# openclimatefix/predict_pv_yield

Measured on AMD Instinct MI355X. Metric: PV-site samples/sec (train step), conv3d 12->6 frames, higher is better.
Workload: dtype bf16; 1 GPU; conv3d train step (fwd + NMAE + bwd + Adam): sat [B,11,18,64,64] N(0,1), 4x Conv3d(3x3x3, 32ch) + fc 128/128/64, 128.6 M params; per_gpu_batch=32, global_batch=32, t_frames=18, parallelism=single

## Files before the change

predict_pv_yield_amd/csrc/conv3d_wgrad_bf16_v2.hip:

```cpp
#include "pv_common.h"

namespace pv {

constexpr int W2TR = 8, W2TRI = 10, W2TW = 32, W2XW = 34;
constexpr int W2_SLAB_ELEMS = 28 * 32 * 32;
constexpr uint32_t W2_INVALID = 0x40000000u;

typedef __attribute__((address_space(3))) s16x4 w2_lds_s16x4;
typedef __attribute__((address_space(3))) unsigned char* w2_lds_ptr;
typedef int w2_i32x4 __attribute__((ext_vector_type(4)));

__device__ __forceinline__ void w2_lds_dma16(uint32_t lds_addr, uint32_t voff, w2_i32x4 rsrc, uint32_t soff) {
  asm volatile("s_mov_b32 m0, %0\n\ts_nop 0\n\tbuffer_load_dwordx4 %1, %2, %3 offen lds" ::"s"(lds_addr), "v"(voff), "s"(rsrc),
               "s"(soff)
               : "memory");
}
__device__ __forceinline__ w2_i32x4 w2_rsrc(const void* base, int bytes) {
  const uintptr_t a = (uintptr_t)base;
  return (w2_i32x4){(int)(uint32_t)a, (int)((a >> 32) & 0xffffu), bytes, 0x00020000};
}

#ifdef PV_DIAG_STAMPS
__device__ unsigned long long wgrad2_diag[PV_DIAG_WAVES * PV_DIAG_SLOTS];
#endif

template <int NACC, int Q>
__device__ __forceinline__ void w2_interleave() {
  if constexpr (Q < NACC) {
    constexpr int R = 2 + 2 * NACC;
    __builtin_amdgcn_sched_group_barrier(0x008, 1, 0);
    __builtin_amdgcn_sched_group_barrier(0x100, R / NACC + (Q < R % NACC ? 1 : 0), 0);
    w2_interleave<NACC, Q + 1>();
  }
}

template <int CPAD, bool F16 = false, bool PACK12 = false>
__global__ __launch_bounds__(512, 2) void conv3d_wgrad_bf16_v2_kernel(
    const uint16_t* __restrict__ x, const uint16_t* __restrict__ dy, float* __restrict__ slabs, int t_in, int h_in, int w_in,
    int t_out, int h_out, int w_out, int pad_t, int pad_h, int pad_w, int n_colblk, int t_chunk, int rpb) {
  constexpr int NCH = CPAD / 8;
  constexpr int VPR = 16 / NCH;
  constexpr int VOXB = CPAD * 2;
  constexpr int ROWB = W2XW * VOXB;
  constexpr int SLOTB = W2TRI * ROWB;
  constexpr int XVPP = 1024 / VOXB;
  constexpr int XPIECES = (W2XW + XVPP - 1) / XVPP;
  constexpr int XTAIL_LANES = (W2XW - (XPIECES - 1) * XVPP) * NCH;
  constexpr int DROWB = W2TW * 64;
  constexpr int DSLOTB = W2TR * DROWB;
  constexpr int NXS = 5;
  __shared__ __attribute__((aligned(1024))) unsigned char lds[NXS * SLOTB + 256 + 2 * DSLOTB];
  unsigned char* lds_const = lds + NXS * SLOTB;
  unsigned char* lds_dy = lds_const + 256;

  const int tid = threadIdx.x;
  const int lane = tid & 63;
  const int wave8 = __builtin_amdgcn_readfirstlane(tid >> 6);
  const bool loader = wave8 >= 4;
  const int wave = wave8 & 3;
  const int grp = lane >> 4;
  const int qi = (lane & 15) >> 2;
  const int pi = lane & 3;
  const int hh = grp >> 1;
  const int cb = 16 * (grp & 1);

  const int h0 = blockIdx.x * rpb;
  const int b = blockIdx.z;
  const int tc0 = blockIdx.y * t_chunk;
  const int tc1 = min(tc0 + t_chunk, t_out);
  const int wg_id = (blockIdx.z * gridDim.y + blockIdx.y) * gridDim.x + blockIdx.x;
  float* slab = slabs + (size_t)wg_id * W2_SLAB_ELEMS;

  static_assert(!PACK12 || CPAD == 16, "PACK12 packs the 16-channel image");
  constexpr bool PAIRED = CPAD == 16;
  constexpr int NACC = PACK12 ? 3 : (PAIRED ? 4 : 7);
  f32x16 acc[NACC];
#pragma unroll
  for (int i = 0; i < NACC; ++i)
#pragma unroll
    for (int j = 0; j < 16; ++j) acc[i][j] = 0.f;

  const int nt = tc1 - tc0, tn = nt + 2;
  const int n_items = nt > 0 ? nt * n_colblk : 0;
  const int u_end = tn * n_colblk;
  const uint32_t lds_base = __builtin_amdgcn_readfirstlane((uint32_t)(uintptr_t)(w2_lds_ptr)lds);

  if (n_items > 0 && loader) {
    const uint32_t x_plane_b = (uint32_t)h_in * w_in * CPAD * 2u, x_row_b = (uint32_t)w_in * CPAD * 2u;
    const uint32_t d_plane_b = (uint32_t)h_out * w_out * 64u, d_row_b = (uint32_t)w_out * 64u;
    const size_t x_sample = (size_t)t_in * h_in * w_in * CPAD, d_sample = (size_t)t_out * h_out * w_out * 32;
    const void* const x_base = x + (size_t)b * x_sample;
    const void* const d_base = dy + (size_t)b * d_sample;
    const int x_bytes = (int)(x_sample * 2), d_bytes = (int)(d_sample * 2);
    uint32_t xrow_src[3];
    bool xrow_in[3];
#pragma unroll
    for (int i = 0; i < 3; ++i) {
      const int hi = h0 - pad_h + wave + 4 * i;
      xrow_in[i] = (unsigned)hi < (unsigned)h_in && wave + 4 * i < rpb + 2;
      xrow_src[i] = xrow_in[i] ? (uint32_t)hi * x_row_b : 0u;
    }
    uint32_t drow_src[2];
    bool drow_in[2];
#pragma unroll
    for (int i = 0; i < 2; ++i) {
      const int ho = h0 + wave + 4 * i;
      drow_in[i] = ho < h_out && wave + 4 * i < rpb;
      drow_src[i] = drow_in[i] ? (uint32_t)ho * d_row_b : 0u;
    }
    const bool has_third_row = wave + 8 < W2TRI;
    auto x_slice = [&](int u) {
      const int cb = u / tn, s = tc0 + (u - cb * tn), w0 = cb * W2TW;
      const int ti = s - pad_t;
      const bool t_ok = (unsigned)ti < (unsigned)t_in;
      const uint32_t slot = lds_base + (uint32_t)((u % NXS) * SLOTB);
#pragma unroll
      for (int pc = 0; pc < XPIECES; ++pc) {
        const int v = pc * XVPP + lane / NCH;
        const int src = (lane % NCH) ^ ((v / VPR) % NCH);
        const int wi = w0 - pad_w + v;
        const uint32_t lane_off = ((unsigned)wi < (unsigned)w_in && v < W2XW) ? (uint32_t)(wi * CPAD + src * 8) * 2u : W2_INVALID;
#pragma unroll
        for (int i = 0; i < 3; ++i) {
          if (i == 2 && !has_third_row) continue;
          const bool ok = t_ok && xrow_in[i];
          if (pc + 1 < XPIECES || lane < XTAIL_LANES)
            w2_lds_dma16(slot + (uint32_t)((wave + 4 * i) * ROWB + pc * 1024), lane_off, w2_rsrc(x_base, ok ? x_bytes : 0),
                         ok ? (uint32_t)ti * x_plane_b + xrow_src[i] : 0u);
        }
      }
    };
    auto d_slice = [&](int v_seq) {
      const int cb = v_seq / nt, t = tc0 + (v_seq - cb * nt), w0 = cb * W2TW;
      const uint32_t slot = lds_base + (uint32_t)(NXS * SLOTB + 256 + (v_seq & 1) * DSLOTB);
#pragma unroll
      for (int pc = 0; pc < 2; ++pc) {
        const int v = pc * 16 + (lane >> 2);
        const int src = (lane & 3) ^ ((v >> 2) & 3);
        const uint32_t lane_off = (w0 + v) < w_out ? (uint32_t)((w0 + v) * 32 + src * 8) * 2u : W2_INVALID;
#pragma unroll
        for (int i = 0; i < 2; ++i) {
          const bool ok = drow_in[i];
          w2_lds_dma16(slot + (uint32_t)((wave + 4 * i) * DROWB + pc * 1024), lane_off, w2_rsrc(d_base, ok ? d_bytes : 0),
                       ok ? (uint32_t)t * d_plane_b + drow_src[i] : 0u);
        }
      }
    };

    int next_u = 0;
    for (; next_u < 4 && next_u < u_end; ++next_u) x_slice(next_u);
    d_slice(0);
    for (int j = 0; j < n_items; ++j) {
      const int cb = j / nt, u0 = cb * tn + (j - cb * nt);
      __builtin_amdgcn_s_waitcnt(0x0f70);
      __syncthreads();
      if (next_u < u0 + 3) {
        for (; next_u < u0 + 3; ++next_u) x_slice(next_u);
        __builtin_amdgcn_s_waitcnt(0x0f70);
        __syncthreads();
      }
      for (; next_u <= u0 + 4 && next_u < u_end; ++next_u) x_slice(next_u);
      if (j + 1 < n_items) d_slice(j + 1);
    }
  } else if (n_items > 0) {
    if (tid < 64) reinterpret_cast<uint32_t*>(lds_const)[tid] = tid < 32 ? (F16 ? 0x3c003c00u : 0x3f803f80u) : 0u;

    int aoff[2];
#pragma unroll
    for (int s = 0; s < 2; ++s) {
      const int v = 8 * hh + 4 * s + qi;
      const int chunk = (cb + 4 * pi) >> 3;
      aoff[s] = v * 64 + ((chunk ^ ((v >> 2) & 3)) << 4) + (pi & 1) * 8;
    }
    int boff[NACC][2];
    int bkt[NACC];
    int my_tap[NACC];
#pragma unroll
    for (int i = 0; i < NACC; ++i) {
      int tap, c4 = 0;
      if constexpr (PACK12) {
        const int piece = 8 * (wave + 4 * i) + 4 * (grp & 1) + pi;
        tap = piece / 3;
        c4 = piece - 3 * tap;
        if (piece > 81) tap = 28;
      } else {
        tap = PAIRED ? 2 * (wave + 4 * i) + (grp & 1) : wave + 4 * i;
      }
      my_tap[i] = tap;
      if (tap > 26) tap = 26;
      const int kt = tap / 9, kh = (tap / 3) % 3, kw = tap % 3;
      bkt[i] = kt;
      const int cbx = PAIRED ? 0 : cb;
#pragma unroll
      for (int s = 0; s < 2; ++s) {
        const int v = kw + 8 * hh + 4 * s + qi;
        const int chunk = PACK12 ? (c4 >> 1) : ((cbx + 4 * pi) >> 3);
        const int sub = PACK12 ? (c4 & 1) : (pi & 1);
        boff[i][s] = kh * ROWB + v * VOXB + ((chunk ^ ((v / VPR) % NCH)) << 4) + sub * 8;
      }
    }
    typedef __attribute__((ext_vector_type(8))) short s16x8;
    const int last_tap = (PAIRED || PACK12) ? my_tap[NACC - 1] : (wave == 3 ? 27 : 0);
    const unsigned char* const_frag = last_tap < 27 ? nullptr : lds_const + (last_tap == 27 ? 0 : 128) + (lane & 15) * 8;

#ifdef PV_DIAG_STAMPS
    unsigned long long dg[PV_DIAG_SLOTS] = {0, 0, 0, 0, 0, 0, 0, 0}, s0, s1, s2;
#endif
    for (int j = 0; j < n_items; ++j) {
      const int cbj = j / nt, u0 = cbj * tn + (j - cbj * nt);
      PV_STAMP(s0);
      __syncthreads();
      if (cbj > 0 && j == cbj * nt) __syncthreads();
      PV_STAMP(s1);
      int slot_of_kt[3];
#pragma unroll
      for (int kt = 0; kt < 3; ++kt) slot_of_kt[kt] = ((u0 + kt) % NXS) * SLOTB;
      const unsigned char* dy_slot = lds_dy + (j & 1) * DSLOTB;
      int bslot[NACC];
#pragma unroll
      for (int i = 0; i < NACC; ++i) bslot[i] = bkt[i] == 0 ? slot_of_kt[0] : (bkt[i] == 1 ? slot_of_kt[1] : slot_of_kt[2]);
      auto read_step = [&](int st, s16x4 (&ra)[2], s16x4 (&rb)[NACC][2]) {
        const int rho = st >> 1, cg = st & 1;
        const unsigned char* ap = dy_slot + rho * DROWB + cg * 16 * 64;
        ra[0] = __builtin_amdgcn_ds_read_tr16_b64_v4i16((w2_lds_s16x4*)(ap + aoff[0]));
        ra[1] = __builtin_amdgcn_ds_read_tr16_b64_v4i16((w2_lds_s16x4*)(ap + aoff[1]));
        const int xo = rho * ROWB + cg * 16 * VOXB;
#pragma unroll
        for (int i = 0; i < NACC; ++i) {
          const unsigned char* bp = lds + bslot[i] + xo;
          const unsigned char* p0 = bp + boff[i][0];
          const unsigned char* p1 = bp + boff[i][1];
          if (i == NACC - 1) {
            p0 = const_frag ? const_frag : p0;
            p1 = const_frag ? const_frag : p1;
          }
          rb[i][0] = __builtin_amdgcn_ds_read_tr16_b64_v4i16((w2_lds_s16x4*)p0);
          rb[i][1] = __builtin_amdgcn_ds_read_tr16_b64_v4i16((w2_lds_s16x4*)p1);
        }
      };
      auto mfma_step = [&](const s16x4 (&ra)[2], const s16x4 (&rb)[NACC][2]) {
        const s16x8 a8 = {ra[0][0], ra[0][1], ra[0][2], ra[0][3], ra[1][0], ra[1][1], ra[1][2], ra[1][3]};
        typedef _Float16 w2_f16x8 __attribute__((ext_vector_type(8)));
#pragma unroll
        for (int i = 0; i < NACC; ++i) {
          s16x8 t8 = {rb[i][0][0], rb[i][0][1], rb[i][0][2], rb[i][0][3], rb[i][1][0], rb[i][1][1], rb[i][1][2], rb[i][1][3]};
          if constexpr (F16)
            acc[i] = __builtin_amdgcn_mfma_f32_32x32x16_f16(__builtin_bit_cast(w2_f16x8, a8), __builtin_bit_cast(w2_f16x8, t8), acc[i], 0, 0, 0);
          else
            acc[i] = __builtin_amdgcn_mfma_f32_32x32x16_bf16(__builtin_bit_cast(bf16x8, a8), __builtin_bit_cast(bf16x8, t8), acc[i], 0, 0, 0);
        }
      };
      s16x4 ra0[2], ra1[2], rb0[NACC][2], rb1[NACC][2];
      const bool skip_last_row = rpb < W2TR;
      read_step(0, ra0, rb0);
#pragma unroll
      for (int st = 0; st < W2TR * 2; st += 2) {
        if (st == W2TR * 2 - 2 && skip_last_row) break;
        __builtin_amdgcn_sched_barrier(0);
        read_step(st + 1, ra1, rb1);
        mfma_step(ra0, rb0);
        w2_interleave<NACC, 0>();
        __builtin_amdgcn_sched_barrier(0);
        if (st + 2 < W2TR * 2) {
          read_step(st + 2, ra0, rb0);
          mfma_step(ra1, rb1);
          w2_interleave<NACC, 0>();
        } else {
          mfma_step(ra1, rb1);
        }
        __builtin_amdgcn_sched_barrier(0);
      }
#ifdef PV_DIAG_STAMPS
      PV_STAMP(s2);
      dg[0] += s1 - s0;
      dg[1] += s2 - s1;
      dg[2] += 1;
#endif
    }
#ifdef PV_DIAG_STAMPS
    if (lane == 0 && wg_id * 4 + wave < PV_DIAG_WAVES)
      for (int i = 0; i < PV_DIAG_SLOTS; ++i) wgrad2_diag[(size_t)(wg_id * 4 + wave) * PV_DIAG_SLOTS + i] = dg[i];
#endif
  }
  if (loader) return;

  const int half = lane >> 5;
#pragma unroll
  for (int i = 0; i < NACC; ++i) {
    int tapslot = PAIRED ? 2 * (wave + 4 * i) + ((lane & 31) >> 4) : wave + 4 * i;
    int ci = PAIRED ? (lane & 15) : (lane & 31);
    if constexpr (PACK12) {
      const int piece = 8 * (wave + 4 * i) + ((lane & 31) >> 2);
      tapslot = piece / 3;
      ci = 4 * (piece - 3 * tapslot) + (lane & 3);
      if (piece > 81) tapslot = 28;
    }
    if (tapslot <= 27) {
      float* dst = slab + (size_t)tapslot * 1024 + ci;
#pragma unroll
      for (int j = 0; j < 16; ++j) {
        const int co = (j & 3) + 8 * (j >> 2) + 4 * half;
        dst[co * 32] = acc[i][j];
      }
    }
  }
}

void wgrad_v2_grid(const pv_conv3d_dims* d, int* n_rowblk, int* n_colblk, int* n_tchunk, int* t_chunk, int* rows_per_blk) {
  const int to = d->t_in + 2 * d->pad_t - 2, ho = d->h_in + 2 * d->pad_h - 2, wo = d->w_in + 2 * d->pad_w - 2;
  *n_rowblk = (ho + W2TR - 1) / W2TR;
  if ((long long)d->batch * *n_rowblk < 256 && (long long)d->batch * (*n_rowblk + 1) <= 256 &&
      (ho + *n_rowblk) / (*n_rowblk + 1) < (ho + *n_rowblk - 1) / *n_rowblk)
    *n_rowblk += 1;
  *rows_per_blk = (ho + *n_rowblk - 1) / *n_rowblk;
  *n_colblk = (wo + W2TW - 1) / W2TW;
  const long long tiles = (long long)d->batch * *n_rowblk;
  int max_chunks = (to + 1) / 2;
  if (max_chunks < 1) max_chunks = 1;
  int ntc = 1;
  long long best = -1;
  for (int c = 1; c <= max_chunks && tiles * c <= 16 * 256; ++c) {
    const int tch = (to + c - 1) / c, nch = (to + tch - 1) / tch;
    const long long rounds = (tiles * nch + 255) / 256;
    const long long cost = rounds * (tch + 2);
    if (best < 0 || cost < best) best = cost, ntc = nch;
  }
  *t_chunk = (to + ntc - 1) / ntc;
  *n_tchunk = (to + *t_chunk - 1) / *t_chunk;
}

size_t wgrad_v2_workspace_bytes(const pv_conv3d_dims* d) {
  int nrb, ncb, ntc, tch, rpb;
  wgrad_v2_grid(d, &nrb, &ncb, &ntc, &tch, &rpb);
  return (size_t)d->batch * nrb * ntc * W2_SLAB_ELEMS * sizeof(float);
}

int launch_conv3d_wgrad_bf16_v2(const uint16_t* x, const uint16_t* dy, float* slabs, const pv_conv3d_dims* d, int to, int ho,
                                int wo, hipStream_t st, int* n_slabs, bool f16) {
  if (((uintptr_t)x % 16) != 0 || ((uintptr_t)dy % 16) != 0) return 1;
  int nrb, ncb, ntc, tch, rpb;
  wgrad_v2_grid(d, &nrb, &ncb, &ntc, &tch, &rpb);
  *n_slabs = d->batch * nrb * ntc;
  dim3 grid((unsigned)nrb, (unsigned)ntc, (unsigned)d->batch);
#define PV_W2(CP, HALF)                                                                                                       \
  hipLaunchKernelGGL((conv3d_wgrad_bf16_v2_kernel<CP, HALF>), grid, dim3(512), 0, st, x, dy, slabs, d->t_in, d->h_in, d->w_in, to, \
                     ho, wo, d->pad_t, d->pad_h, d->pad_w, ncb, tch, rpb)
#define PV_W2P(HALF)                                                                                                        \
  hipLaunchKernelGGL((conv3d_wgrad_bf16_v2_kernel<16, HALF, true>), grid, dim3(512), 0, st, x, dy, slabs, d->t_in, d->h_in, d->w_in, \
                     to, ho, wo, d->pad_t, d->pad_h, d->pad_w, ncb, tch, rpb)
  if (pv_bf16_cpad(d->c_in) == 16) {
    const bool pack12 = d->c_in <= 12 && !getenv("PV_WGRAD_NO_PACK12");
    if (pack12) { if (f16) PV_W2P(true); else PV_W2P(false); }
    else { if (f16) PV_W2(16, true); else PV_W2(16, false); }
  } else { if (f16) PV_W2(32, true); else PV_W2(32, false); }
#undef PV_W2P
#undef PV_W2
  return 0;
}


constexpr int WR_GROUPS = 16;
__global__ __launch_bounds__(64 * WR_GROUPS) void conv3d_wgrad_reduce_kernel(const float* __restrict__ slabs, int n_slabs,
                                                                              float* __restrict__ dw, float* __restrict__ dbias,
                                                                              int c_out, int c_in) {
  __shared__ float part[WR_GROUPS][64];
  const int lane = threadIdx.x & 63, grp = threadIdx.x >> 6;
  const int i = blockIdx.x * 64 + lane;
  float s0 = 0.f, s1 = 0.f, s2 = 0.f, s3 = 0.f;
  for (int k = grp; k < n_slabs; k += 16 * WR_GROUPS) {
    float v[16];
#pragma unroll
    for (int j = 0; j < 16; ++j) v[j] = (k + WR_GROUPS * j < n_slabs) ? slabs[(size_t)(k + WR_GROUPS * j) * W2_SLAB_ELEMS + i] : 0.f;
#pragma unroll
    for (int j = 0; j < 16; j += 4) s0 += v[j], s1 += v[j + 1], s2 += v[j + 2], s3 += v[j + 3];
  }
  part[grp][lane] = (s0 + s1) + (s2 + s3);
  __syncthreads();
  if (grp == 0) {
    float t[WR_GROUPS];
#pragma unroll
    for (int q = 0; q < WR_GROUPS; ++q) t[q] = part[q][lane];
#pragma unroll
    for (int w = WR_GROUPS / 2; w >= 1; w >>= 1)
#pragma unroll
      for (int q = 0; q < w; ++q) t[q] = t[2 * q] + t[2 * q + 1];
    const float s = t[0];
    const int tap = i >> 10, co = (i >> 5) & 31, ci = i & 31;
    if (tap < 27) {
      if (dw && co < c_out && ci < c_in) dw[((size_t)co * c_in + ci) * 27 + tap] = s;
    } else if (dbias && ci == 0 && co < c_out) {
      dbias[co] = s;
    }
  }
}

__global__ __launch_bounds__(256) void wgrad_gate_copy_kernel(const u32x4* __restrict__ dy, const u32x4* __restrict__ y,
                                                              u32x4* __restrict__ dst, size_t n8) {
  const size_t stride = (size_t)gridDim.x * blockDim.x;
  for (size_t i = (size_t)blockIdx.x * blockDim.x + threadIdx.x; i < n8; i += stride) {
    const u32x4 g = dy[i], a = y[i];
    u32x4 o;
#pragma unroll
    for (int j = 0; j < 4; ++j) o[j] = g[j] & (relu_pair01(a[j]) * 0xffffu);
    dst[i] = o;
  }
}

}

using namespace pv;

extern "C" {

int pv_conv3d_bwd_weight_bf16_workspace_bytes(const pv_conv3d_dims* d, size_t* bytes) {
  PV_REQUIRE(d && bytes, PV_EINVAL, "pv_conv3d_bwd_weight_bf16_workspace_bytes: null pointer");
  PV_REQUIRE(d->batch > 0 && d->t_in > 0 && d->h_in > 0 && d->w_in > 0, PV_EINVAL,
             "pv_conv3d_bwd_weight_bf16_workspace_bytes: bad dims");
  const long long to = d->t_in + 2 * d->pad_t - 2, ho = d->h_in + 2 * d->pad_h - 2, wo = d->w_in + 2 * d->pad_w - 2;
  const size_t dy_bytes = (to > 0 && ho > 0 && wo > 0) ? (size_t)d->batch * to * ho * wo * pv_bf16_cpad(d->c_out) * 2 : 0;
  *bytes = ((wgrad_v2_workspace_bytes(d) + 255) & ~(size_t)255) + dy_bytes;
  return PV_OK;
}

int pv_conv3d_bwd_weight_bf16(const uint16_t* x, const uint16_t* dy, const uint16_t* y_relu_mask, float* dw,
                              float* dbias, const pv_conv3d_dims* d, void* workspace, size_t workspace_bytes,
                              void* stream) {
  PV_REQUIRE(d && x && dy && workspace, PV_EINVAL, "pv_conv3d_bwd_weight_bf16: null pointer");
  PV_REQUIRE(d->batch > 0 && d->c_in > 0 && d->c_in <= 32 && d->c_out > 0 && d->c_out <= 32, PV_ESIZE,
             "pv_conv3d_bwd_weight_bf16: channels (%d -> %d) must be in 1..32", d->c_in, d->c_out);
  PV_REQUIRE(d->pad_t >= 0 && d->pad_t <= 2 && d->pad_h >= 0 && d->pad_h <= 2 && d->pad_w >= 0 && d->pad_w <= 2,
             PV_EINVAL, "pv_conv3d_bwd_weight_bf16: padding must be 0..2");
  const int to = d->t_in + 2 * d->pad_t - 2, ho = d->h_in + 2 * d->pad_h - 2, wo = d->w_in + 2 * d->pad_w - 2;
  PV_REQUIRE(to > 0 && ho > 0 && wo > 0, PV_ESIZE, "pv_conv3d_bwd_weight_bf16: input smaller than the kernel");
  PV_REQUIRE(d->batch <= 65535, PV_ESIZE, "pv_conv3d_bwd_weight_bf16: batch too large for grid.z");
  PV_REQUIRE((size_t)d->t_in * d->h_in * d->w_in * 64 <= 0x40000000ull, PV_ESIZE,
             "pv_conv3d_bwd_weight_bf16: one sample exceeds 1 GiB (buffer-addressing limit of this kernel)");
  const size_t slab_bytes = (wgrad_v2_workspace_bytes(d) + 255) & ~(size_t)255;
  PV_REQUIRE(workspace_bytes >= wgrad_v2_workspace_bytes(d), PV_ESIZE, "pv_conv3d_bwd_weight_bf16: workspace too small");
  PV_REQUIRE(((uintptr_t)x % 16) == 0 && ((uintptr_t)dy % 16) == 0 && ((uintptr_t)workspace % 16) == 0, PV_EINVAL,
             "pv_conv3d_bwd_weight_bf16: x, dy and the workspace must be 16-byte aligned");
  hipStream_t st = as_stream(stream);
  if (y_relu_mask) {
    const size_t n = (size_t)d->batch * to * ho * wo * pv_bf16_cpad(d->c_out);
    PV_REQUIRE(workspace_bytes >= slab_bytes + n * 2, PV_ESIZE,
               "pv_conv3d_bwd_weight_bf16: a gate needs room for the gated copy of dY behind the slabs (workspace_bytes query)");
    PV_REQUIRE(((uintptr_t)y_relu_mask % 16) == 0, PV_EINVAL, "pv_conv3d_bwd_weight_bf16: the gate must be 16-byte aligned");
    uint16_t* gated = reinterpret_cast<uint16_t*>(static_cast<char*>(workspace) + slab_bytes);
    hipLaunchKernelGGL(wgrad_gate_copy_kernel, dim3(stream_grid(n / 8, 256)), dim3(256), 0, st,
                       reinterpret_cast<const u32x4*>(dy), reinterpret_cast<const u32x4*>(y_relu_mask),
                       reinterpret_cast<u32x4*>(gated), n / 8);
    dy = gated;
  }
  int n2 = 0;
  PV_REQUIRE(launch_conv3d_wgrad_bf16_v2(x, dy, (float*)workspace, d, to, ho, wo, st, &n2, false) == 0, PV_EINVAL,
             "pv_conv3d_bwd_weight_bf16: x and dy must be 16-byte aligned");
  hipLaunchKernelGGL(conv3d_wgrad_reduce_kernel, dim3(W2_SLAB_ELEMS / 64), dim3(64 * WR_GROUPS), 0, st, (const float*)workspace, n2,
                     dw, dbias, d->c_out, d->c_in);
  return check_launch("pv_conv3d_bwd_weight_bf16");
}

int pv_conv3d_bwd_weight_f16(const uint16_t* x, const uint16_t* dy, float* dw, float* dbias, const pv_conv3d_dims* d,
                             void* workspace, size_t workspace_bytes, void* stream) {
  PV_REQUIRE(d && x && dy && workspace, PV_EINVAL, "pv_conv3d_bwd_weight_f16: null pointer");
  PV_REQUIRE(d->batch > 0 && d->c_in > 0 && d->c_in <= 32 && d->c_out > 0 && d->c_out <= 32, PV_ESIZE,
             "pv_conv3d_bwd_weight_f16: channels (%d -> %d) must be in 1..32", d->c_in, d->c_out);
  PV_REQUIRE(d->pad_t >= 0 && d->pad_t <= 2 && d->pad_h >= 0 && d->pad_h <= 2 && d->pad_w >= 0 && d->pad_w <= 2,
             PV_EINVAL, "pv_conv3d_bwd_weight_f16: padding must be 0..2");
  const int to = d->t_in + 2 * d->pad_t - 2, ho = d->h_in + 2 * d->pad_h - 2, wo = d->w_in + 2 * d->pad_w - 2;
  PV_REQUIRE(to > 0 && ho > 0 && wo > 0, PV_ESIZE, "pv_conv3d_bwd_weight_f16: input smaller than the kernel");
  PV_REQUIRE(d->batch <= 65535, PV_ESIZE, "pv_conv3d_bwd_weight_f16: batch too large for grid.z");
  PV_REQUIRE((size_t)d->t_in * d->h_in * d->w_in * 64 <= 0x40000000ull, PV_ESIZE,
             "pv_conv3d_bwd_weight_f16: one sample exceeds 1 GiB (buffer-addressing limit of this kernel)");
  PV_REQUIRE(workspace_bytes >= wgrad_v2_workspace_bytes(d), PV_ESIZE, "pv_conv3d_bwd_weight_f16: workspace too small");
  hipStream_t st = as_stream(stream);
  int n2 = 0;
  PV_REQUIRE(launch_conv3d_wgrad_bf16_v2(x, dy, (float*)workspace, d, to, ho, wo, st, &n2, true) == 0, PV_EINVAL,
             "pv_conv3d_bwd_weight_f16: x and dy must be 16-byte aligned");
  hipLaunchKernelGGL(conv3d_wgrad_reduce_kernel, dim3(W2_SLAB_ELEMS / 64), dim3(64 * WR_GROUPS), 0, st, (const float*)workspace, n2,
                     dw, dbias, d->c_out, d->c_in);
  return check_launch("pv_conv3d_bwd_weight_f16");
}

}

#ifdef PV_DIAG_STAMPS
extern "C" int pv_diag_read_wgrad2(unsigned long long* host, size_t n) {
  return hipMemcpyFromSymbol(host, HIP_SYMBOL(pv::wgrad2_diag), n * sizeof(unsigned long long)) == hipSuccess ? 0 : -1;
}
#endif
```

Before: 21100 samples/s.

## Share x fragments across kh taps in 32-channel conv3d wgrad kernel

Adds a KHS variant of the bf16 wgrad kernel for 32-channel inputs. Each compute wave now owns two (kt,kw) groups across all three kh offsets and marches over input rows, so one x-row fragment read from LDS feeds three kh accumulators and dy rows are held in a three-deep register ring. This is meant to cut LDS read traffic per MFMA. In exchange it adds more register pressure, a fully compile-time unrolled step schedule with custom MFMA/read interleaving, and a new tap-to-accumulator mapping that must match the slab writeback. The path is on by default for CPAD=32 and can be disabled with an environment variable.

```diff
diff --git a/predict_pv_yield_amd/csrc/conv3d_wgrad_bf16_v2.hip b/predict_pv_yield_amd/csrc/conv3d_wgrad_bf16_v2.hip
--- a/predict_pv_yield_amd/csrc/conv3d_wgrad_bf16_v2.hip
+++ b/predict_pv_yield_amd/csrc/conv3d_wgrad_bf16_v2.hip
@@ -34,7 +34,43 @@
   }
 }
 
-template <int CPAD, bool F16 = false, bool PACK12 = false>
+template <int V>
+struct w2_c { static constexpr int v = V; };
+__host__ __device__ constexpr int w2_khs_rows(bool skip) { return skip ? W2TR - 1 : W2TR; }
+__host__ __device__ constexpr int w2_khs_steps(bool skip) { return 2 * (w2_khs_rows(skip) + 2); }
+__host__ __device__ constexpr int w2_khs_mfmas(int st, bool skip) {
+  const int ir = st >> 1, rows = w2_khs_rows(skip);
+  int n = ir < rows ? 1 : 0;
+  for (int kh = 0; kh < 3; ++kh) n += (ir - kh >= 0 && ir - kh < rows) ? 2 : 0;
+  return n;
+}
+__host__ __device__ constexpr int w2_khs_reads(int st, bool skip, bool ones) {
+  const int ir = st >> 1, rows = w2_khs_rows(skip);
+  return st >= w2_khs_steps(skip) ? 0 : (ir < rows + 2 ? 4 : 0) + (ir < rows ? (ones ? 2 : 4) : 0);
+}
+__host__ __device__ constexpr int w2_khs_tap(int wave, int i) {
+  if (i == 6) return wave < 3 ? 20 + 3 * wave : 27;
+  const int g = 2 * wave + i / 3, kh = i % 3;
+  return 9 * (g / 3) + 3 * kh + g % 3;
+}
+template <int NM, int NR, int Q = 0>
+__device__ __forceinline__ void w2_interleave_n() {
+  if constexpr (Q < NM && NR > 0) {
+    __builtin_amdgcn_sched_group_barrier(0x008, 1, 0);
+    if constexpr (NR / NM + (Q < NR % NM ? 1 : 0) > 0)
+      __builtin_amdgcn_sched_group_barrier(0x100, NR / NM + (Q < NR % NM ? 1 : 0), 0);
+    w2_interleave_n<NM, NR, Q + 1>();
+  }
+}
+template <int ST, int END, class F, class SK, class ON>
+__device__ __forceinline__ void w2_khs_run(F& f, SK sk, ON on) {
+  if constexpr (ST < END) {
+    f(w2_c<ST>{}, sk, on);
+    w2_khs_run<ST + 1, END>(f, sk, on);
+  }
+}
+
+template <int CPAD, bool F16 = false, bool PACK12 = false, bool KHS = false>
 __global__ __launch_bounds__(512, 2) void conv3d_wgrad_bf16_v2_kernel(
     const uint16_t* __restrict__ x, const uint16_t* __restrict__ dy, float* __restrict__ slabs, int t_in, int h_in, int w_in,
     int t_out, int h_out, int w_out, int pad_t, int pad_h, int pad_w, int n_colblk, int t_chunk, int rpb) {
@@ -72,6 +108,7 @@
   float* slab = slabs + (size_t)wg_id * W2_SLAB_ELEMS;
 
   static_assert(!PACK12 || CPAD == 16, "PACK12 packs the 16-channel image");
+  static_assert(!KHS || CPAD == 32, "the kh-sharing march needs one tap per accumulator");
   constexpr bool PAIRED = CPAD == 16;
   constexpr int NACC = PACK12 ? 3 : (PAIRED ? 4 : 7);
   f32x16 acc[NACC];
@@ -202,10 +239,24 @@
     typedef __attribute__((ext_vector_type(8))) short s16x8;
     const int last_tap = (PAIRED || PACK12) ? my_tap[NACC - 1] : (wave == 3 ? 27 : 0);
     const unsigned char* const_frag = last_tap < 27 ? nullptr : lds_const + (last_tap == 27 ? 0 : 128) + (lane & 15) * 8;
+    int goff[3][2];
+    int gkt[3];
+#pragma unroll
+    for (int f = 0; f < 3; ++f) {
+      const int g = f < 2 ? 2 * wave + f : 8;
+      const int kw = g % 3;
+      gkt[f] = g / 3;
+#pragma unroll
+      for (int s = 0; s < 2; ++s) {
+        const int v = kw + 8 * hh + 4 * s + qi;
+        goff[f][s] = (f == 2 && wave < 3 ? wave * ROWB : 0) + v * VOXB + ((((cb + 4 * pi) >> 3) ^ ((v / VPR) % NCH)) << 4) + (pi & 1) * 8;
+      }
+    }
 
 #ifdef PV_DIAG_STAMPS
     unsigned long long dg[PV_DIAG_SLOTS] = {0, 0, 0, 0, 0, 0, 0, 0}, s0, s1, s2;
 #endif
+    auto run_items = [&](auto ones_c, auto skip_c) {
     for (int j = 0; j < n_items; ++j) {
       const int cbj = j / nt, u0 = cbj * tn + (j - cbj * nt);
       PV_STAMP(s0);
@@ -216,6 +267,69 @@
 #pragma unroll
       for (int kt = 0; kt < 3; ++kt) slot_of_kt[kt] = ((u0 + kt) % NXS) * SLOTB;
       const unsigned char* dy_slot = lds_dy + (j & 1) * DSLOTB;
+      typedef _Float16 w2_f16x8 __attribute__((ext_vector_type(8)));
+      auto mfma1 = [&](f32x16& c, const s16x4 (&a)[2], const s16x4 (&t)[2]) {
+        const s16x8 a8 = {a[0][0], a[0][1], a[0][2], a[0][3], a[1][0], a[1][1], a[1][2], a[1][3]};
+        const s16x8 t8 = {t[0][0], t[0][1], t[0][2], t[0][3], t[1][0], t[1][1], t[1][2], t[1][3]};
+        if constexpr (F16)
+          c = __builtin_amdgcn_mfma_f32_32x32x16_f16(__builtin_bit_cast(w2_f16x8, a8), __builtin_bit_cast(w2_f16x8, t8), c, 0, 0, 0);
+        else
+          c = __builtin_amdgcn_mfma_f32_32x32x16_bf16(__builtin_bit_cast(bf16x8, a8), __builtin_bit_cast(bf16x8, t8), c, 0, 0, 0);
+      };
+      if constexpr (KHS) {
+        const unsigned char* xp[3][2];
+        const unsigned char* ap[2];
+#pragma unroll
+        for (int s = 0; s < 2; ++s) {
+          ap[s] = dy_slot + aoff[s];
+#pragma unroll
+          for (int f = 0; f < 3; ++f)
+            xp[f][s] = lds + (gkt[f] == 0 ? slot_of_kt[0] : (gkt[f] == 1 ? slot_of_kt[1] : slot_of_kt[2])) + goff[f][s];
+        }
+        s16x4 xf[2][3][2], dyw[3][2][2], onesf[2];
+        auto read_khs = [&](auto st_c, auto skip_c, auto ones_c) {
+          constexpr int ST = decltype(st_c)::v, IR = ST >> 1, CG = ST & 1, ROWS = w2_khs_rows(decltype(skip_c)::v);
+          constexpr int xo = IR * ROWB + CG * 16 * VOXB;
+          if constexpr (IR < ROWS + 2) {
+#pragma unroll
+            for (int f = 0; f < 2; ++f)
+#pragma unroll
+              for (int s = 0; s < 2; ++s) xf[ST & 1][f][s] = __builtin_amdgcn_ds_read_tr16_b64_v4i16((w2_lds_s16x4*)(xp[f][s] + xo));
+          }
+          if constexpr (IR < ROWS) {
+#pragma unroll
+            for (int s = 0; s < 2; ++s) {
+              dyw[IR % 3][CG][s] = __builtin_amdgcn_ds_read_tr16_b64_v4i16((w2_lds_s16x4*)(ap[s] + IR * DROWB + CG * 16 * 64));
+              if constexpr (!decltype(ones_c)::v)
+                xf[ST & 1][2][s] = __builtin_amdgcn_ds_read_tr16_b64_v4i16((w2_lds_s16x4*)(xp[2][s] + xo));
+            }
+          }
+        };
+        auto step_khs = [&](auto st_c, auto skip_c, auto ones_c) {
+          constexpr int ST = decltype(st_c)::v, IR = ST >> 1, CG = ST & 1;
+          constexpr bool SKIP = decltype(skip_c)::v, ONES = decltype(ones_c)::v;
+          constexpr int ROWS = w2_khs_rows(SKIP);
+          __builtin_amdgcn_sched_barrier(0);
+          if constexpr (ST + 1 < w2_khs_steps(SKIP)) read_khs(w2_c<ST + 1>{}, skip_c, ones_c);
+#pragma unroll
+          for (int f = 0; f < 2; ++f)
+#pragma unroll
+            for (int kh = 0; kh < 3; ++kh)
+              if (IR - kh >= 0 && IR - kh < ROWS) mfma1(acc[3 * f + kh], dyw[(IR - kh + 3) % 3][CG], xf[ST & 1][f]);
+          if constexpr (IR < ROWS) {
+            if constexpr (ONES) mfma1(acc[6], dyw[IR % 3][CG], onesf);
+            else mfma1(acc[6], dyw[IR % 3][CG], xf[ST & 1][2]);
+          }
+          w2_interleave_n<w2_khs_mfmas(ST, SKIP), w2_khs_reads(ST + 1, SKIP, ONES)>();
+          __builtin_amdgcn_sched_barrier(0);
+        };
+        if constexpr (decltype(ones_c)::v) {
+          onesf[0] = __builtin_amdgcn_ds_read_tr16_b64_v4i16((w2_lds_s16x4*)const_frag);
+          onesf[1] = __builtin_amdgcn_ds_read_tr16_b64_v4i16((w2_lds_s16x4*)const_frag);
+        }
+        read_khs(w2_c<0>{}, skip_c, ones_c);
+        w2_khs_run<0, w2_khs_steps(decltype(skip_c)::v)>(step_khs, skip_c, ones_c);
+      } else {
       int bslot[NACC];
 #pragma unroll
       for (int i = 0; i < NACC; ++i) bslot[i] = bkt[i] == 0 ? slot_of_kt[0] : (bkt[i] == 1 ? slot_of_kt[1] : slot_of_kt[2]);
@@ -270,6 +384,7 @@
         }
         __builtin_amdgcn_sched_barrier(0);
       }
+      }
 #ifdef PV_DIAG_STAMPS
       PV_STAMP(s2);
       dg[0] += s1 - s0;
@@ -277,6 +392,18 @@
       dg[2] += 1;
 #endif
     }
+    };
+    if constexpr (KHS) {
+      if (rpb < W2TR) {
+        if (wave == 3) run_items(w2_c<1>{}, w2_c<1>{});
+        else run_items(w2_c<0>{}, w2_c<1>{});
+      } else {
+        if (wave == 3) run_items(w2_c<1>{}, w2_c<0>{});
+        else run_items(w2_c<0>{}, w2_c<0>{});
+      }
+    } else {
+      run_items(w2_c<0>{}, w2_c<0>{});
+    }
 #ifdef PV_DIAG_STAMPS
     if (lane == 0 && wg_id * 4 + wave < PV_DIAG_WAVES)
       for (int i = 0; i < PV_DIAG_SLOTS; ++i) wgrad2_diag[(size_t)(wg_id * 4 + wave) * PV_DIAG_SLOTS + i] = dg[i];
@@ -287,7 +414,7 @@
   const int half = lane >> 5;
 #pragma unroll
   for (int i = 0; i < NACC; ++i) {
-    int tapslot = PAIRED ? 2 * (wave + 4 * i) + ((lane & 31) >> 4) : wave + 4 * i;
+    int tapslot = PAIRED ? 2 * (wave + 4 * i) + ((lane & 31) >> 4) : (KHS ? w2_khs_tap(wave, i) : wave + 4 * i);
     int ci = PAIRED ? (lane & 15) : (lane & 31);
     if constexpr (PACK12) {
       const int piece = 8 * (wave + 4 * i) + ((lane & 31) >> 2);
@@ -348,11 +475,17 @@
 #define PV_W2P(HALF)                                                                                                        \
   hipLaunchKernelGGL((conv3d_wgrad_bf16_v2_kernel<16, HALF, true>), grid, dim3(512), 0, st, x, dy, slabs, d->t_in, d->h_in, d->w_in, \
                      to, ho, wo, d->pad_t, d->pad_h, d->pad_w, ncb, tch, rpb)
+#define PV_W2K(HALF)                                                                                                        \
+  hipLaunchKernelGGL((conv3d_wgrad_bf16_v2_kernel<32, HALF, false, true>), grid, dim3(512), 0, st, x, dy, slabs, d->t_in, d->h_in, \
+                     d->w_in, to, ho, wo, d->pad_t, d->pad_h, d->pad_w, ncb, tch, rpb)
   if (pv_bf16_cpad(d->c_in) == 16) {
     const bool pack12 = d->c_in <= 12 && !getenv("PV_WGRAD_NO_PACK12");
     if (pack12) { if (f16) PV_W2P(true); else PV_W2P(false); }
     else { if (f16) PV_W2(16, true); else PV_W2(16, false); }
+  } else if (!getenv("PV_WGRAD_NO_KH_SHARE")) {
+    if (f16) PV_W2K(true); else PV_W2K(false);
   } else { if (f16) PV_W2(32, true); else PV_W2(32, false); }
+#undef PV_W2K
 #undef PV_W2P
 #undef PV_W2
   return 0;
```

New measurement: 20780 samples/s. 0.985x the previous value.
